# cornellius-gp/linear_operator

Hardware: AMD Instinct MI355X
Metric: cg_member_matvecs_per_sec (higher is better)
Workload: dtype f32

## Files before the change

### linear_operator_amd/csrc/lo_cg_close.h

```cpp
#pragma once
#include "lo_device.h"
#include "lo_internal.h"
#include "lo_cg_onchip.h"
#include "lo_group_reduce.h"

namespace lo {

__device__ __forceinline__ void cg_close_solve(const OnchipArgs& a, const int ngroups, const int t) {
  __shared__ int closer_s;
  __shared__ float red_s[R4_TPB];
  if (t == 0) closer_s = (atomicAdd(a.close_count, 1) == ngroups - 1) ? 1 : 0;
  __syncthreads();
  if (closer_s) {
    float lsum = 0.f, lnan = 0.f, lnotconv = 0.f, lredo = 0.f;
    unsigned spin = 0;
    bool lost = false;
    for (int64_t i = t; i < a.B && !lost; i += R4_TPB) {
      unsigned long long gr;
      for (;;) {
        gr = granule_load(a.close_gran + i);
        if ((granule_tag(gr) & ~7u) == a.close_epoch) break;
        if (++spin > kHandoffMaxSpin || __hip_atomic_load(a.err, __ATOMIC_RELAXED, __HIP_MEMORY_SCOPE_AGENT) != 0) {
          lost = true;
          break;
        }
        __builtin_amdgcn_s_sleep(1);
      }
      if (lost) break;
      const float rn = granule_value(gr);
      const unsigned fl = granule_tag(gr);
      lsum += rn;
      if (rn != rn || (fl & 2u)) lnan = 1.f;
      if (!(fl & 1u)) lnotconv = 1.f;
      if (fl & 4u) lredo = 1.f;
    }
    if (lost) atomicExch(a.err, 1);
    const float mean = block_sum256(lsum, red_s) / (float)a.B;
    const float anynan = block_sum256(lnan, red_s);
    const float notconv = block_sum256(lnotconv, red_s);
    const float redo = block_sum256(lredo, red_s);
    if (t == 0) {
      CgCtrl* c = a.close_ctrl;
      const bool nan = anynan > 0.f;
      const bool skip = !nan && notconv == 0.f;
      const bool tol = !nan && !skip && a.close_floor_ok && mean < a.close_tol;
      c->rs_redo = redo > 0.f ? 1 : 0;
      c->iterations = skip ? 0 : a.iters;
      c->mean_resid = mean;
      c->nan_detected = nan ? 1 : 0;
      c->skipped = skip ? 1 : 0;
      c->tol_reached = tol ? 1 : 0;
      c->stop = (nan || skip || tol) ? 1 : 0;
      c->last_tridiag_iter = 0;
      c->tri_disabled = 0;
      c->oc_err = __hip_atomic_load(a.err, __ATOMIC_RELAXED, __HIP_MEMORY_SCOPE_AGENT);
      if (a.handoff_owned) {
        c->oc_next = c->oc_next_ls = c->pf_next = 0;
        __hip_atomic_store(a.next_member, 0, __ATOMIC_RELAXED, __HIP_MEMORY_SCOPE_AGENT);
        __hip_atomic_store(a.close_count, 0, __ATOMIC_RELAXED, __HIP_MEMORY_SCOPE_AGENT);
      }
      if (a.close_mirror) {
        *a.close_mirror = *c;
        __threadfence_system();
        __hip_atomic_store(reinterpret_cast<unsigned*>(a.close_mirror) + 63, a.close_ticket, __ATOMIC_RELEASE,
                           __HIP_MEMORY_SCOPE_SYSTEM);
      }
    }
  }
}

}
```

### linear_operator_amd/csrc/lo_rspace3.hip

```cpp
#include <algorithm>
#include <atomic>
#include <mutex>
#include <type_traits>
#include <stdlib.h>

#include "lo_device.h"
#include "lo_internal.h"
#include "lo_cg_onchip.h"
#include "lo_group_reduce.h"
#include "lo_cg_close.h"
#include "lo_f64_lanes.h"

namespace lo {

namespace {

typedef float f32x4 __attribute__((ext_vector_type(4)));
typedef __attribute__((address_space(1))) const f32x4 g_cf4;
typedef __attribute__((address_space(1))) const float g_cf;
typedef __attribute__((address_space(1))) float g_f;
typedef __attribute__((address_space(1))) const char g_cc;
template <class T>
__device__ __forceinline__ T* opaque_uniform(T* p) {
  asm volatile("" : "+s"(p));
  return p;
}

constexpr int R3_TPB = 256;
constexpr int R3_ROWS = 1024;

struct PeerOut {
  float* buf[7];
  int n;
  long long member_off;
};
PeerOut g_peer_out = {{nullptr, nullptr, nullptr, nullptr, nullptr, nullptr, nullptr}, 0, 0};
std::mutex g_peer_mu;

__host__ __device__ constexpr int r3_np(int RC) { return 2 * RC + 6; }

__device__ __forceinline__ unsigned xor4_dpp_u(unsigned x) {
  const int a = __builtin_amdgcn_update_dpp(0, (int)x, 0x104, 0xf, 0x5, false);
  return (unsigned)__builtin_amdgcn_update_dpp(a, (int)x, 0x114, 0xf, 0xa, false);
}
__device__ __forceinline__ double halve4_d(double lo, double hi, int lane) {
  const bool up = (lane & 4) != 0;
  const double keep = up ? hi : lo;
  const double send = up ? lo : hi;
  return keep + mk_d(xor4_dpp_u(lo_w(send)), xor4_dpp_u(hi_w(send)));
}

template <int CH>
__device__ __forceinline__ double rows_reduce_d(double (&p)[CH], int lane) {
  if constexpr (CH == 8) {
#pragma unroll
    for (int m = 0; m < 4; ++m) p[m] = halve4_d(p[m], p[m + 4], lane);
    p[0] = halve_pair_d<2>(p[0], p[2], lane);
    p[1] = halve_pair_d<2>(p[1], p[3], lane);
    return halve_pair_d<1>(p[0], p[1], lane);
  } else if constexpr (CH == 4) {
    p[0] = halve_pair_d<2>(p[0], p[2], lane);
    p[1] = halve_pair_d<2>(p[1], p[3], lane);
    return halve_pair_d<1>(p[0], p[1], lane);
  } else {
    return halve_pair_d<1>(p[0], p[1], lane);
  }
}

template <int RC, int GW>
__global__ __launch_bounds__(R3_TPB, 2) void k_cg_rspace3(OnchipArgs a, PeerOut po) {
  constexpr int CH = RC / 4;
  constexpr int RPI = 64 / CH;
  constexpr int NI = 256 / RPI;
  constexpr int NP = r3_np(RC);
  constexpr int MLD = RC + 2;
  constexpr int NH = RC / 2;
  constexpr int NG = 2 * GW * NP;
  __shared__ __attribute__((aligned(16))) float bst[4][256];
  __shared__ __attribute__((aligned(16))) float dst[4][256];
  __shared__ __attribute__((aligned(16))) double mat_s[3 * RC * MLD];
  __shared__ __attribute__((aligned(16))) double red[4][NP];
  __shared__ __attribute__((aligned(16))) double res[NP];
  __shared__ __attribute__((aligned(16))) double gv[4][32];
  __shared__ unsigned polw[GW > 1 ? NG : 2];
  const GroupPlace gp = group_place(GW, (int)gridDim.x / 8);
  if (!gp.active) return;
  const int grp = gp.grp, wig = gp.wig, ngroups = gp.ngroups;
  const int t = threadIdx.x, lane = t & 63, wave = t >> 6;
  const int wave_u = __builtin_amdgcn_readfirstlane(wave);
  unsigned long long* const gbase = a.gbuf + (size_t)grp * 2 * NG;
  unsigned tag = a.tag_base;
  bool same_xcd = false;
  const unsigned xcc = xcc_id();
  bool first = true;
  const int row0 = wig * R3_ROWS + 256 * wave_u;
  const int row0c = max(0, min(row0, a.N - 256));
  const bool di_full = a.dinv_mode == LO_DIAG_FULL;
  float* const bw = bst[wave_u];
  float* const dw = dst[wave_u];
  constexpr int NPF = 8;
  f32x4 pre[NPF];
  constexpr int NXT = NI - NPF;
  f32x4 nxt[NXT > 0 ? NXT : 1];
  auto request = [&](int64_t bm, int tl_, int i_lo, auto cnt, f32x4* dst) {
    const int ln_ = tl_ & 63, k_ = ln_ & (CH - 1), g_ = ln_ / CH;
    const unsigned loff = (unsigned)((g_ * RC + 4 * k_) * sizeof(float));
    g_cc* Cw = (g_cc*)(a.C + ((size_t)bm * a.N + row0c) * RC);
#pragma unroll
    for (int q = 0; q < decltype(cnt)::value / 8; ++q) {
      g_cc* bq = opaque_uniform(Cw + (i_lo + 8 * q + 4) * 1024);
#pragma unroll
      for (int i = 0; i < 8; ++i) dst[8 * q + i] = *(g_cf4*)(bq + loff + (i - 4) * 1024);
    }
  };
  int64_t b = grp;
  {
    int tl0 = t;
    asm volatile("" : "+v"(tl0));
    if (b < a.B) {
      request(b, tl0, 0, std::integral_constant<int, NPF>{}, pre);
      request(b, tl0, NPF, std::integral_constant<int, NXT>{}, nxt);
    } else {
#pragma unroll
      for (int i = 0; i < NPF; ++i) pre[i] = (f32x4){0.f, 0.f, 0.f, 0.f};
    }
  }
  while (b < a.B) {
    const bool stamp = a.dbg && b == a.dbg_member && wig == 0 && t == 0;
    if (stamp) a.dbg[0] = wall_clock64();
    int drawn = 0;
    if (wig == 0 && t == 0) drawn = atomicAdd(a.next_member, 1);
    int tl = t;
    asm volatile("" : "+v"(tl));
    const int ln = tl & 63, k = ln & (CH - 1), g = ln / CH;
    f32x4 Cr[NI];
#pragma unroll
    for (int i = 0; i < NPF; ++i) Cr[i] = pre[i];
#pragma unroll
    for (int i = 0; i < NXT; ++i) Cr[NPF + i] = nxt[i];
    float bq4[4], dq4[4];
    {
      g_cf* bb_ = opaque_uniform((g_cf*)(a.rhs + (size_t)b * a.N + row0c));
      g_cf* dd_ = opaque_uniform((g_cf*)(di_full ? a.dinv + (size_t)b * a.N + row0c : a.dinv + b));
      const int lo_e = row0 - row0c, hi_e = max(0, min(256, a.N - row0c));
      const int dstride = di_full ? 1 : 0;
#pragma unroll
      for (int m = 0; m < 4; ++m) {
        const int e = ln + 64 * m;
        const bool own = e >= lo_e && e < hi_e;
        bq4[m] = own ? bb_[e] : 0.f;
        dq4[m] = own ? dd_[e * dstride] : 0.f;
      }
    }
    constexpr int NM = (3 * RC * RC / 2 + R3_TPB - 1) / R3_TPB;
    f32x4 mv[NM];
    {
      typedef __attribute__((address_space(1))) const f32x4 g_m4;
      const g_m4* src = (const g_m4*)(a.RSD + (size_t)b * 6 * RC * RC);
#pragma unroll
      for (int u = 0; u < NM; ++u) {
        const int e = min(tl + R3_TPB * u, 3 * RC * RC / 2 - 1);
        const int ms = e / (RC * RC / 2);
        const int mg = ms == 0 ? 0 : ms + 1;
        mv[u] = src[(size_t)mg * (RC * RC / 2) + (e - ms * (RC * RC / 2))];
      }
    }
    const double lam_mine = a.RSD[((size_t)b * 6 + 5) * RC * RC + min(ln & 31, RC - 1)];
#pragma unroll
    for (int m = 0; m < 4; ++m) {
      bw[ln + 64 * m] = bq4[m];
      dw[ln + 64 * m] = dq4[m];
    }
#pragma unroll
    for (int u = 0; u < NM; ++u) {
      const int e = tl + R3_TPB * u;
      if (e < 3 * RC * RC / 2) {
        const int mi = e / (RC / 2), jj = e % (RC / 2);
        *reinterpret_cast<f32x4*>(&mat_s[mi * MLD + 2 * jj]) = mv[u];
      }
    }
    __builtin_amdgcn_wave_barrier();
    if (stamp) a.dbg[1] = wall_clock64();

    {
      double aw[4] = {0.0, 0.0, 0.0, 0.0}, au[4] = {0.0, 0.0, 0.0, 0.0};
#pragma unroll
      for (int i0 = 0; i0 < NI; i0 += 4) {
#pragma unroll
        for (int i = i0; i < i0 + 4; ++i) {
          const int r = RPI * i + g;
          const double bb = (double)bw[r];
          const double bd = bb * (double)dw[r];
          const double c0 = (double)Cr[i].x, c1 = (double)Cr[i].y, c2 = (double)Cr[i].z, c3 = (double)Cr[i].w;
          aw[0] = fma(c0, bd, aw[0]); au[0] = fma(c0, bb, au[0]);
          aw[1] = fma(c1, bd, aw[1]); au[1] = fma(c1, bb, au[1]);
          aw[2] = fma(c2, bd, aw[2]); au[2] = fma(c2, bb, au[2]);
          aw[3] = fma(c3, bd, aw[3]); au[3] = fma(c3, bb, au[3]);
        }
        __builtin_amdgcn_sched_barrier(0);
      }
      double s_acc = 0.0, a_acc = 0.0, d2_acc = 0.0;
#pragma unroll
      for (int j = 0; j < 4; ++j) {
        const int rw = 64 * j + RPI * k + g;
        const double bb = (double)bw[rw], di = (double)dw[rw];
        s_acc = fma(bb, bb * di, s_acc);
        a_acc = fma(bb, bb, a_acc);
        d2_acc = fma(di, di, d2_acc);
      }
      double h0 = halve_pair_d<32>(aw[0], au[0], ln), h1 = halve_pair_d<32>(aw[1], au[1], ln);
      double h2 = halve_pair_d<32>(aw[2], au[2], ln), h3 = halve_pair_d<32>(aw[3], au[3], ln);
      h0 = halve_pair_d<16>(h0, h2, ln);
      h1 = halve_pair_d<16>(h1, h3, ln);
      double mine = halve_pair_d<8>(h0, h1, ln);
      if constexpr (CH <= 4) mine = bfly_add_d<4>(mine);
      if constexpr (CH <= 2) mine = bfly_add_d<2>(mine);
      const int comp = (((ln >> 4) & 1) << 1) | ((ln >> 3) & 1);
      const bool writer = (ln & 7 & ~(CH - 1)) == 0;
      if (writer) red[wave_u][((ln >> 5) ? RC : 0) + 4 * k + comp] = mine;
      const double ssum = wave_sum_fast_d(s_acc), asum = wave_sum_fast_d(a_acc), d2sum = wave_sum_fast_d(d2_acc);
      if (ln == 0) {
        red[wave_u][2 * RC] = ssum;
        red[wave_u][2 * RC + 1] = asum;
        red[wave_u][2 * RC + 2] = (wig == 0 && wave_u == 0) ? (double)(ngroups + drawn) : 0.0;
        red[wave_u][2 * RC + 3] = d2sum;
        unsigned xc = xcc;
        asm volatile("" : "+s"(xc));
        red[wave_u][2 * RC + 4] = (first && wave_u == 0) ? (double)xc : 0.0;
        red[wave_u][2 * RC + 5] = (first && wave_u == 0) ? (double)(xc * xc) : 0.0;
      }
    }
#pragma unroll
    for (int i = 0; i < NI; ++i) asm volatile("" : "+v"(Cr[i]));
    __builtin_amdgcn_sched_barrier(0);
    if (a.prefetch & 4) __builtin_amdgcn_s_setprio(3);
    {
      ++tag;
      int tt = (int)threadIdx.x;
      asm volatile("" : "+v"(tt));
      __syncthreads();
      if constexpr (GW == 1) {
        if (tt < NP) res[tt] = (red[0][tt] + red[1][tt]) + (red[2][tt] + red[3][tt]);
      } else {
        unsigned long long* slot = gbase + (size_t)(tag & 1u) * NG;
        if (tt < NP) {
          const double v = (red[0][tt] + red[1][tt]) + (red[2][tt] + red[3][tt]);
          unsigned long long* mine = slot + ((size_t)wig * NP + tt) * 2;
          granule_store(mine, granule_pack_bits(tag, lo_w(v)), same_xcd);
          granule_store(mine + 1, granule_pack_bits(tag, hi_w(v)), same_xcd);
        }
        constexpr int PER = (NG + R3_TPB - 1) / R3_TPB;
        constexpr int CKQ = PER < 8 ? PER : 8;
        unsigned spin = 0;
        bool lost = false;
#pragma unroll 1
        for (int q0 = 0; q0 < PER && !lost; q0 += CKQ) {
          unsigned long long x[CKQ];
          for (;;) {
            bool ok = true;
#pragma unroll
            for (int q = 0; q < CKQ; ++q) {
              const int idx = tt + R3_TPB * (q0 + q);
              x[q] = granule_load(slot + min(idx, NG - 1));
              ok = ok && (granule_tag(x[q]) == tag);
            }
            if (ok) break;
            if (poll_give_up(spin, a.err)) {
              lost = true;
              break;
            }
            __builtin_amdgcn_s_sleep(1);
          }
#pragma unroll
          for (int q = 0; q < CKQ; ++q) {
            const int idx = tt + R3_TPB * (q0 + q);
            if (idx < NG) polw[idx] = granule_bits(x[q]);
          }
        }
        __syncthreads();
        if (tt < NP) {
          double tot = 0.0;
#pragma unroll
          for (int w = 0; w < GW; ++w) tot += mk_d(polw[(w * NP + tt) * 2], polw[(w * NP + tt) * 2 + 1]);
          res[tt] = tot;
        }
      }
      __syncthreads();
    }
    if (GW > 1 && first) {
      unsigned xc = xcc;
      asm volatile("" : "+s"(xc));
      same_xcd = same_xcd_verdict(res[2 * RC + 4], res[2 * RC + 5], GW, xc, a.allow_l2_handoff);
    }
    first = false;
    if (stamp) a.dbg[2] = wall_clock64();
    const int64_t b_next = (int64_t)res[2 * RC + 2];
    {
      int tp = t;
      asm volatile("" : "+v"(tp));
      if (b_next < a.B) {
        request(b_next, tp, 0, std::integral_constant<int, NPF>{}, pre);
      } else {
#pragma unroll
        for (int i = 0; i < NPF; ++i) pre[i] = (f32x4){0.f, 0.f, 0.f, 0.f};
      }
    }
    if (a.prefetch & 1) __builtin_amdgcn_s_setprio(3);

    const int j = lane & 31, hf = lane >> 5;
    const bool live = j < RC;
    const int jr = live ? j : RC - 1;
    double yj = 0.0, xi = 0.0;
    float nrm;
    {
      double a0 = res[2 * RC + 1], s = res[2 * RC];
      const double d2 = res[2 * RC + 3];
      nrm = sqrtf((float)a0);
      const bool rhs_zero = nrm < a.eps;
      if (rhs_zero) nrm = 1.0f;
      const double inv = 1.0 / (double)nrm;
      const double w0 = live ? res[jr] * inv : 0.0, u0 = live ? res[RC + jr] * inv : 0.0;
      s *= inv * inv;
      a0 *= inv * inv;
      float sa = a.stop_after;
      asm volatile("" : "+s"(sa));
      const double sure_rz = 2.0 * (double)sa * (double)sa * sqrt(d2);
      auto own_row_dot = [&](const double* mrow, const double* vec) {
        double a0_ = 0.0, a1_ = 0.0;
#pragma unroll
        for (int q = 0; q < NH; q += 2) {
          const double2 xa = *reinterpret_cast<const double2*>(mrow + q);
          const double2 xx = *reinterpret_cast<const double2*>(vec + q);
          a0_ = fma(xa.x, xx.x, a0_);
          a1_ = fma(xa.y, xx.y, a1_);
        }
        double lo_, up_;
        halves_d(a0_ + a1_, lo_, up_);
        return lo_ + up_;
      };
      double* myv = gv[wave];
      if (hf == 0) myv[j] = w0;
      __builtin_amdgcn_wave_barrier();
      const double* row0m = mat_s + (size_t)jr * MLD + hf * NH;
      double c0 = own_row_dot(row0m, myv + hf * NH);
      double e0 = own_row_dot(row0m + (size_t)1 * RC * MLD, myv + hf * NH);
      const double* nrow = row0m + (size_t)2 * RC * MLD;
      const double* tucol = mat_s + (size_t)(1 * RC + hf * NH) * MLD + jr;
      c0 = live ? c0 : 0.0;
      e0 = live ? e0 : 0.0;
      double tau2 = s - lanes32_sum_d(c0 * e0);
      tau2 = tau2 > 0.0 ? tau2 : 0.0;
      const bool delicate = !rhs_zero && tau2 < 1e-2 * s;
      const double lam = live ? lam_mine : 1.0;
      long long ts_a = 0, ts_b = 0;
      if (stamp) ts_a = wall_clock64();
      double cj = c0, qj = 0.0, etaj = 0.0;
      double cp = 1.0, qp = 0.0, etap = 0.0;
      double rz = 0.0, pApE = 0.0, alpha = 0.0, beta = 0.0;
      float rn = 0.f, last_alpha = 0.f;
      bool conv = false;
      unsigned close_flags = 0u;
      const size_t bc = (size_t)b;
      const bool rec = wig == 0 && lane == 0;
      const int last_owner = (a.iters - 1) & 3;
      for (int kk = -1; kk < a.iters; ++kk) {
        if (kk >= 0) {
          last_alpha = (float)alpha;
          etaj = fma(alpha, qj, etaj);
          etap = fma(alpha, qp, etap);
          cj = fma(-alpha * lam, qj, cj);
          cp = fma(-alpha, qp, cp);
        }
        const double lc = lam * cj;
        const bool lo_h = hf == 0;
        const float inv_rz = __builtin_amdgcn_rcpf((float)rz);
        const double red2 = row16_sum_d(halve_pair_d<16>(lo_h ? cj * cj : lc * qj, lo_h ? lc * cj : 0.0, lane));
        const auto pick = [&](double v, int ln_) {
          return mk_d((unsigned)__builtin_amdgcn_readlane((int)lo_w(v), ln_),
                      (unsigned)__builtin_amdgcn_readlane((int)hi_w(v), ln_));
        };
        const double cc = pick(red2, 0), clc = pick(red2, 16), clq = pick(red2, 32);
        const double rzn = fma(cp * cp, tau2, cc);
        const bool sure = rzn > sure_rz;
        const bool rec_first = kk == 0 && a.close_gran == nullptr && wave == 0;
        const bool rec_last = kk == a.iters - 1 && wave == last_owner;
        const bool own = rec_first || rec_last || !sure;
        float rnn = 0.f;
        if (kk < 0) {
          const float s1f = (float)a0;
          rnn = __builtin_amdgcn_sqrtf(s1f < 0.f ? 0.f : s1f);
        } else if (own) {
          const double dl = fma(-cp, c0, cj);
          __builtin_amdgcn_wave_barrier();
          if (hf == 0) myv[j] = dl;
          __builtin_amdgcn_wave_barrier();
          double gj_;
          {
            double a0_ = 0.0, a1_ = 0.0;
#pragma unroll
            for (int q = 0; q < NH; q += 2) {
              const double2 dd = *reinterpret_cast<const double2*>(myv + hf * NH + q);
              a0_ = fma(tucol[(size_t)q * MLD], dd.x, a0_);
              a1_ = fma(tucol[(size_t)(q + 1) * MLD], dd.y, a1_);
            }
            double lo_, up_;
            halves_d(a0_ + a1_, lo_, up_);
            gj_ = live ? lo_ + up_ : 0.0;
          }
          __builtin_amdgcn_wave_barrier();
          if (hf == 0) myv[j] = gj_;
          __builtin_amdgcn_wave_barrier();
          const double nd = own_row_dot(nrow, myv + hf * NH);
          const double r2 = row16_sum_d(halve_pair_d<16>(gj_ * nd, gj_ * u0, lane));
          const double dnd = pick(r2, 0), dm = pick(r2, 16);
          const double s1 = fma(cp, fma(cp, a0, 2.0 * dm), dnd);
          const float s1f = (float)s1;
          rnn = __builtin_amdgcn_sqrtf(s1f < 0.f ? 0.f : s1f);
        }
        if (kk >= 0) {
          beta = ((float)rz < a.eps) ? 0.0 : (double)((float)rzn * inv_rz);
          if (rhs_zero) rnn = 0.f;
          rn = rnn;
          if (rec && (rec_first || rec_last)) a.resid_rec[(size_t)kk * a.B + bc] = rn;
        } else {
          beta = 0.0;
          rn = rnn;
          if (wig == 0 && t == 0) a.init_conv[bc] = (rn < a.stop_after) ? 1 : 0;
          close_flags = ((rn < a.stop_after) ? 1u : 0u) | (delicate ? 4u : 0u);
          if (delicate && rec && wave == 0) atomicOr(a.err + 4, 1);
        }
        if (kk == 0 && (rnn != rnn || rzn != rzn)) close_flags |= 2u;
        conv = (own || rhs_zero) ? (rn < a.stop_after) : false;
        rz = rzn;
        pApE = fma(beta, fma(beta, pApE, 2.0 * clq), clc);
        qj = fma(beta, qj, cj);
        qp = fma(beta, qp, cp);
        const double pAp = fma(qp * qp, tau2, pApE);
        alpha = ((float)pAp < a.eps) ? 0.0 : (double)((float)rz * __builtin_amdgcn_rcpf((float)pAp));
        if (conv) alpha = 0.0;
      }
      if (stamp) ts_b = wall_clock64();
      if (rec && wave == last_owner) {
        a.rhs_norm[bc] = nrm;
        a.rhs_is_zero[bc] = rhs_zero ? 1 : 0;
        a.rz[bc] = (float)rz;
        a.alpha[bc] = last_alpha;
        a.beta[bc] = (float)beta;
        a.resid_norm[bc] = rn;
        a.has_conv[bc] = conv ? 1 : 0;
        if (a.close_gran) {
          granule_store(a.close_gran + b, granule_pack(a.close_epoch | close_flags, rn), false);
        }
      }
      __builtin_amdgcn_wave_barrier();
      if (hf == 0) myv[j] = fma(-etap, e0, etaj);
      __builtin_amdgcn_wave_barrier();
      xi = etap;
      {
        const double* col = mat_s + (size_t)(hf * NH) * MLD + jr;
        double a0_ = 0.0, a1_ = 0.0;
#pragma unroll
        for (int q = 0; q < NH; q += 2) {
          const double2 ee = *reinterpret_cast<const double2*>(myv + hf * NH + q);
          a0_ = fma(col[(size_t)q * MLD], ee.x, a0_);
          a1_ = fma(col[(size_t)(q + 1) * MLD], ee.y, a1_);
        }
        double lo_, up_;
        halves_d(a0_ + a1_, lo_, up_);
        yj = lo_ + up_;
      }
      yj = live ? yj : 0.0;
      if (stamp) {
        a.dbg[5] = ts_a - a.dbg[2];
        a.dbg[6] = ts_b - ts_a;
        a.dbg[7] = wall_clock64() - ts_b;
      }
      __builtin_amdgcn_wave_barrier();
      if (hf == 0) myv[j] = yj * (double)nrm;
      __builtin_amdgcn_wave_barrier();
    }
    if (!(a.prefetch & 2)) __builtin_amdgcn_s_setprio(0);
    if (stamp) a.dbg[3] = wall_clock64();
    {
      int l2 = lane;
      asm volatile("" : "+v"(l2));
      const int k2 = l2 & (CH - 1), g2 = l2 / CH;
      const double* myv = gv[wave];
      const double2 ya = *reinterpret_cast<const double2*>(&myv[4 * k2]);
      const double2 yb = *reinterpret_cast<const double2*>(&myv[4 * k2 + 2]);
      g_f* const xb = opaque_uniform((g_f*)(a.xout + (size_t)b * a.N + row0c));
      const bool more = b_next < a.B;
      g_cc* const Cn = (g_cc*)(a.C + ((size_t)(more ? b_next : b) * a.N + row0c) * RC);
      const unsigned loffn = (unsigned)((g2 * RC + 4 * k2) * sizeof(float));
#pragma unroll
      for (int js = 0; js < 4; ++js) {
        constexpr int J0 = NPF / CH;
        const int jj = (js + J0) & 3;
        double p[CH];
#pragma unroll
        for (int m = 0; m < CH; ++m) {
          const f32x4 c4 = Cr[CH * jj + m];
          p[m] = fma((double)c4.w, yb.y, fma((double)c4.z, yb.x, fma((double)c4.y, ya.y, (double)c4.x * ya.x)));
        }
        const double xv = rows_reduce_d<CH>(p, l2);
        const int rw = 64 * jj + RPI * k2 + g2;
        const int row = row0c + rw;
        const double acc = fma(xi, (double)bw[rw], xv);
        if (row >= row0 && row < a.N) {
          const float xval = (float)(acc * (double)dw[rw]);
          xb[rw] = xval;
          for (int pp = 0; pp < po.n; ++pp)
            ((g_f*)po.buf[pp])[((size_t)(b + po.member_off)) * a.N + row] = xval;
        }
        if (CH * jj >= NPF) {
          g_cc* bqn = opaque_uniform(Cn + (CH * jj + 4) * 1024);
#pragma unroll
          for (int m = 0; m < CH; ++m)
            nxt[CH * jj - NPF + m] = more ? *(g_cf4*)(bqn + loffn + (m - 4) * 1024) : (f32x4){0.f, 0.f, 0.f, 0.f};
        }
      }
      __builtin_amdgcn_wave_barrier();
    }
    __builtin_amdgcn_s_setprio(0);
    if (stamp) a.dbg[4] = wall_clock64();
    __syncthreads();
    b = b_next;
  }
  if (a.close_gran && wig == 0) cg_close_solve(a, ngroups, t);
}

int rspace3_prio() {
  static const int prio = [] {
    const char* e = getenv("LO_RS_PRIO");
    return e ? atoi(e) : 3;
  }();
  return prio;
}

constexpr size_t HO_MAX_WGS = 2 * 320;
constexpr size_t HO_GRAN_PER_WG = 432;
constexpr size_t HO_MAX_MEMBERS = 65536;
constexpr size_t HO_HEAD_BYTES = 256;
constexpr unsigned HO_TAG_LIMIT = 0xfff00000u;
constexpr unsigned HO_EPOCH_LIMIT = 0x1ffffff0u;
struct HandoffBlock {
  char* buf = nullptr;
  size_t bytes = 0;
  bool failed = false;
  unsigned next_tag = 1, next_epoch = 1;
  unsigned last_launch = 0;
  std::atomic<unsigned> confirmed{0};
  bool force_clear = false;
  unsigned clears = 0, launches = 0;
};
HandoffBlock g_handoff[16];
std::atomic<unsigned> g_handoff_ids{0};

HandoffBlock* handoff_block() {
  int dev = 0;
  if (hipGetDevice(&dev) != hipSuccess || dev < 0 || dev >= 16) return nullptr;
  HandoffBlock& h = g_handoff[dev];
  if (!h.buf && !h.failed) {
    h.bytes = HO_HEAD_BYTES + (HO_MAX_WGS * HO_GRAN_PER_WG + HO_MAX_MEMBERS) * sizeof(unsigned long long);
    if (hipMalloc(&h.buf, h.bytes) != hipSuccess || hipMemset(h.buf, 0, h.bytes) != hipSuccess) {
      (void)hipGetLastError();
      h.buf = nullptr;
      h.failed = true;
    }
  }
  return h.buf ? &h : nullptr;
}

bool handoff_advance(unsigned* next_tag, unsigned* next_epoch, int64_t B, unsigned* tag_base, unsigned* epoch) {
  bool wrap = false;
  const unsigned need = (unsigned)B + 2u;
  if (*next_tag >= HO_TAG_LIMIT - need || *next_epoch >= HO_EPOCH_LIMIT) {
    *next_tag = 1;
    *next_epoch = 1;
    wrap = true;
  }
  *tag_base = *next_tag;
  *epoch = *next_epoch;
  *next_tag += need;
  *next_epoch += 1;
  return wrap;
}

struct OwnedLaunch {
  bool inject;
  unsigned* launch_id;
};

template <int RC, int GW>
int rspace3_go(const OnchipArgs& a, int nwg, const OwnedLaunch* own, hipStream_t st) {
  int per_cu = 0;
  if (LO_OCCUPANCY_CACHED(per_cu, (k_cg_rspace3<RC, GW>), R3_TPB, 0) != hipSuccess || per_cu < 2) return LO_ERR_UNSUPPORTED;
  LO_PROF_BEGIN("cg_onchip", st);
  ResidentLaunch guard(st);
  OnchipArgs a2 = a;
  a2.prefetch = rspace3_prio();
  if (own) {
    hipStreamCaptureStatus cap = hipStreamCaptureStatusNone;
    if (hipStreamIsCapturing(st, &cap) != hipSuccess || cap != hipStreamCaptureStatusNone) {
      (void)hipGetLastError();
      return LO_ERR_UNSUPPORTED;
    }
    HandoffBlock* h = (a.B <= (int64_t)HO_MAX_MEMBERS && (size_t)2 * nwg <= HO_MAX_WGS) ? handoff_block() : nullptr;
    if (!h) return LO_ERR_UNSUPPORTED;
    bool clear = h->force_clear || h->last_launch != h->confirmed.load(std::memory_order_acquire);
    h->force_clear = false;
    clear = handoff_advance(&h->next_tag, &h->next_epoch, a.B, &a2.tag_base, &a2.close_epoch) || clear;
    h->last_launch = g_handoff_ids.fetch_add(1, std::memory_order_relaxed) + 1;
    if (h->last_launch == 0) h->last_launch = g_handoff_ids.fetch_add(1, std::memory_order_relaxed) + 1;
    *own->launch_id = h->last_launch;
    ++h->launches;
    if (clear) {
      ++h->clears;
      const int zrc = zero_span(h->buf, h->bytes, st);
      if (zrc) return zrc;
    }
    a2.close_epoch <<= 3;
    a2.handoff_owned = 1;
    a2.err = reinterpret_cast<int*>(h->buf);
    a2.next_member = a2.err + 1;
    a2.close_count = a2.err + 2;
    a2.gbuf = reinterpret_cast<unsigned long long*>(h->buf + HO_HEAD_BYTES);
    a2.close_gran = a2.gbuf + HO_MAX_WGS * HO_GRAN_PER_WG;
    if (own->inject) LO_HIP_CHECK(hipMemsetAsync(a2.err, 1, 1, st));
  }
  PeerOut po;
  {
    std::lock_guard<std::mutex> lk(g_peer_mu);
    po = g_peer_out;
  }
  hipLaunchKernelGGL((k_cg_rspace3<RC, GW>), dim3(2 * nwg), dim3(R3_TPB), 0, st, a2, po);
  LO_PROF_END(st);
  LO_LAUNCH_CHECK();
  return LO_OK;
}

template <int RC>
int rspace3_gw(const OnchipArgs& a, int nwg, const OwnedLaunch* own, hipStream_t st) {
  switch (a.GW) {
    case 1: return rspace3_go<RC, 1>(a, nwg, own, st);
    case 2: return rspace3_go<RC, 2>(a, nwg, own, st);
    case 4: return rspace3_go<RC, 4>(a, nwg, own, st);
    case 8: return rspace3_go<RC, 8>(a, nwg, own, st);
    case 16: return rspace3_go<RC, 16>(a, nwg, own, st);
    case 32: return rspace3_go<RC, 32>(a, nwg, own, st);
  }
  return LO_ERR_UNSUPPORTED;
}

int rspace3_dispatch(int RC, const OnchipArgs& a, int nwg, const OwnedLaunch* own, hipStream_t st) {
  if (!a.RSD || a.x || a.c != 1 || a.ab_rec || !a.xout || a.GW > 32 || a.N < 256 || (int64_t)a.GW * R3_ROWS < a.N)
    return LO_ERR_UNSUPPORTED;
  if (RC == 32) return rspace3_gw<32>(a, nwg, own, st);
  if (RC == 16) return rspace3_gw<16>(a, nwg, own, st);
  if (RC == 8) return rspace3_gw<8>(a, nwg, own, st);
  return LO_ERR_UNSUPPORTED;
}

}

int rspace3_launch(int RC, const OnchipArgs& a, int nwg, hipStream_t st) { return rspace3_dispatch(RC, a, nwg, nullptr, st); }

int rspace3_launch_owned(int RC, const OnchipArgs& a, int nwg, bool inject, unsigned* launch_id, hipStream_t st) {
  if (!a.close_gran || !a.close_ctrl || !a.close_mirror || a.dbg) return LO_ERR_UNSUPPORTED;
  const OwnedLaunch own = {inject, launch_id};
  return rspace3_dispatch(RC, a, nwg, &own, st);
}

void handoff_launch_confirm(unsigned launch_id) {
  int dev = 0;
  if (hipGetDevice(&dev) != hipSuccess || dev < 0 || dev >= 16) return;
  g_handoff[dev].confirmed.store(launch_id, std::memory_order_release);
}

}

extern "C" int lo_peer_gather_set(float* const* bufs, int n, long long member_offset) {
  if (n < 0 || n > 7 || (n > 0 && !bufs)) return LO_ERR_BADARG;
  std::lock_guard<std::mutex> lk(lo::g_peer_mu);
  for (int i = 0; i < 7; ++i) lo::g_peer_out.buf[i] = i < n ? bufs[i] : nullptr;
  lo::g_peer_out.n = n;
  lo::g_peer_out.member_off = member_offset;
  return LO_OK;
}

extern "C" int lo_resident_handoff_debug(int32_t force_clear, int64_t set_next_tag, int64_t set_next_epoch, uint32_t* out) {
  lo::ResidentLock guard;
  int dev = 0;
  if (hipGetDevice(&dev) != hipSuccess || dev < 0 || dev >= 16) return LO_ERR_BADARG;
  lo::HandoffBlock& h = lo::g_handoff[dev];
  if (set_next_tag > 0xffffffffll || set_next_epoch > 0xffffffffll) return LO_ERR_BADARG;
  if (set_next_tag >= 0) h.next_tag = (unsigned)set_next_tag;
  if (set_next_epoch >= 0) h.next_epoch = (unsigned)set_next_epoch;
  if (force_clear) h.force_clear = true;
  if (out) {
    out[0] = h.next_tag;
    out[1] = h.next_epoch;
    out[2] = h.clears;
    out[3] = h.launches;
  }
  return LO_OK;
}
```

Before: 36.35 million.

## Close CG solve earlier and parallelize closer reduction and control writes

```diff
diff --git a/linear_operator_amd/csrc/lo_cg_close.h b/linear_operator_amd/csrc/lo_cg_close.h
--- a/linear_operator_amd/csrc/lo_cg_close.h
+++ b/linear_operator_amd/csrc/lo_cg_close.h
@@ -1,4 +1,6 @@
 #pragma once
+#include <cstddef>
+
 #include "lo_device.h"
 #include "lo_internal.h"
 #include "lo_cg_onchip.h"
@@ -7,19 +9,36 @@
 namespace lo {
 
 __device__ __forceinline__ void cg_close_solve(const OnchipArgs& a, const int ngroups, const int t) {
+  constexpr int CW = (int)(sizeof(CgCtrl) / sizeof(int));
+  static_assert(sizeof(CgCtrl) == CW * sizeof(int) && CW < 63, "the ticket is word 63 of the pinned block");
   __shared__ int closer_s;
-  __shared__ float red_s[R4_TPB];
+  __shared__ float red_s[R4_WAVES];
+  __shared__ unsigned flag_s[R4_WAVES];
   if (t == 0) closer_s = (atomicAdd(a.close_count, 1) == ngroups - 1) ? 1 : 0;
   __syncthreads();
   if (closer_s) {
-    float lsum = 0.f, lnan = 0.f, lnotconv = 0.f, lredo = 0.f;
+    CgCtrl* c = a.close_ctrl;
+    unsigned keep = 0u;
+    if (t < CW && !a.handoff_owned)
+      keep = __hip_atomic_load(reinterpret_cast<const unsigned*>(c) + t, __ATOMIC_RELAXED, __HIP_MEMORY_SCOPE_AGENT);
+    int err0 = 0;
+    if (t < 64) err0 = __hip_atomic_load(a.err, __ATOMIC_RELAXED, __HIP_MEMORY_SCOPE_AGENT);
+    float lsum = 0.f;
+    unsigned lflags = 0u;
     unsigned spin = 0;
     bool lost = false;
-    for (int64_t i = t; i < a.B && !lost; i += R4_TPB) {
-      unsigned long long gr;
+    constexpr int CK = 4;
+    for (int64_t i0 = t; i0 < a.B && !lost; i0 += CK * R4_TPB) {
+      unsigned long long gr[CK];
       for (;;) {
-        gr = granule_load(a.close_gran + i);
-        if ((granule_tag(gr) & ~7u) == a.close_epoch) break;
+        bool ok = true;
+#pragma unroll
+        for (int q = 0; q < CK; ++q) {
+          const int64_t i = i0 + (int64_t)q * R4_TPB;
+          gr[q] = granule_load(a.close_gran + (i < a.B ? i : a.B - 1));
+          ok = ok && ((granule_tag(gr[q]) & ~7u) == a.close_epoch);
+        }
+        if (ok) break;
         if (++spin > kHandoffMaxSpin || __hip_atomic_load(a.err, __ATOMIC_RELAXED, __HIP_MEMORY_SCOPE_AGENT) != 0) {
           lost = true;
           break;
@@ -27,43 +46,70 @@
         __builtin_amdgcn_s_sleep(1);
       }
       if (lost) break;
-      const float rn = granule_value(gr);
-      const unsigned fl = granule_tag(gr);
-      lsum += rn;
-      if (rn != rn || (fl & 2u)) lnan = 1.f;
-      if (!(fl & 1u)) lnotconv = 1.f;
-      if (fl & 4u) lredo = 1.f;
+#pragma unroll
+      for (int q = 0; q < CK; ++q) {
+        if (i0 + (int64_t)q * R4_TPB < a.B) {
+          const float rn = granule_value(gr[q]);
+          const unsigned fl = granule_tag(gr[q]);
+          lsum += rn;
+          if (rn != rn || (fl & 2u)) lflags |= 1u;
+          if (!(fl & 1u)) lflags |= 2u;
+          if (fl & 4u) lflags |= 4u;
+        }
+      }
     }
-    if (lost) atomicExch(a.err, 1);
-    const float mean = block_sum256(lsum, red_s) / (float)a.B;
-    const float anynan = block_sum256(lnan, red_s);
-    const float notconv = block_sum256(lnotconv, red_s);
-    const float redo = block_sum256(lredo, red_s);
-    if (t == 0) {
-      CgCtrl* c = a.close_ctrl;
-      const bool nan = anynan > 0.f;
-      const bool skip = !nan && notconv == 0.f;
+    if (lost) {
+      atomicExch(a.err, 1);
+      lflags |= 8u;
+    }
+    const float wsum = wave_sum(lsum);
+    const unsigned wflags = (__ballot(lflags & 1u) ? 1u : 0u) | (__ballot(lflags & 2u) ? 2u : 0u) |
+                            (__ballot(lflags & 4u) ? 4u : 0u) | (__ballot(lflags & 8u) ? 8u : 0u);
+    if ((t & 63) == 0) {
+      red_s[t >> 6] = wsum;
+      flag_s[t >> 6] = wflags;
+    }
+    __syncthreads();
+    if (t < 64) {
+      long long nb = a.B;
+      unsigned ticket = a.close_ticket;
+      asm volatile("" : "+s"(nb), "+s"(ticket));
+      const float mean = ((red_s[0] + red_s[1]) + (red_s[2] + red_s[3])) / (float)nb;
+      const unsigned flags = (flag_s[0] | flag_s[1]) | (flag_s[2] | flag_s[3]);
+      const bool nan = (flags & 1u) != 0u;
+      const bool skip = !nan && !(flags & 2u);
       const bool tol = !nan && !skip && a.close_floor_ok && mean < a.close_tol;
-      c->rs_redo = redo > 0.f ? 1 : 0;
-      c->iterations = skip ? 0 : a.iters;
-      c->mean_resid = mean;
-      c->nan_detected = nan ? 1 : 0;
-      c->skipped = skip ? 1 : 0;
-      c->tol_reached = tol ? 1 : 0;
-      c->stop = (nan || skip || tol) ? 1 : 0;
-      c->last_tridiag_iter = 0;
-      c->tri_disabled = 0;
-      c->oc_err = __hip_atomic_load(a.err, __ATOMIC_RELAXED, __HIP_MEMORY_SCOPE_AGENT);
-      if (a.handoff_owned) {
-        c->oc_next = c->oc_next_ls = c->pf_next = 0;
+      const int oc_err = (flags & 8u) ? 1 : err0;
+      unsigned w = keep;
+      bool mine = a.handoff_owned != 0;
+      const auto put = [&](size_t off, unsigned v) {
+        if ((size_t)t * sizeof(int) == off) {
+          w = v;
+          mine = true;
+        }
+      };
+      put(offsetof(CgCtrl, rs_redo), (flags & 4u) ? 1u : 0u);
+      put(offsetof(CgCtrl, iterations), skip ? 0u : (unsigned)a.iters);
+      put(offsetof(CgCtrl, mean_resid), __float_as_uint(mean));
+      put(offsetof(CgCtrl, nan_detected), nan ? 1u : 0u);
+      put(offsetof(CgCtrl, skipped), skip ? 1u : 0u);
+      put(offsetof(CgCtrl, tol_reached), tol ? 1u : 0u);
+      put(offsetof(CgCtrl, stop), (nan || skip || tol) ? 1u : 0u);
+      put(offsetof(CgCtrl, last_tridiag_iter), 0u);
+      put(offsetof(CgCtrl, tri_disabled), 0u);
+      put(offsetof(CgCtrl, oc_err), (unsigned)oc_err);
+      if (t < CW && mine) reinterpret_cast<unsigned*>(c)[t] = w;
+      if (a.handoff_owned && t == 0) {
         __hip_atomic_store(a.next_member, 0, __ATOMIC_RELAXED, __HIP_MEMORY_SCOPE_AGENT);
         __hip_atomic_store(a.close_count, 0, __ATOMIC_RELAXED, __HIP_MEMORY_SCOPE_AGENT);
       }
       if (a.close_mirror) {
-        *a.close_mirror = *c;
+        if (t < CW) reinterpret_cast<unsigned*>(a.close_mirror)[t] = w;
         __threadfence_system();
-        __hip_atomic_store(reinterpret_cast<unsigned*>(a.close_mirror) + 63, a.close_ticket, __ATOMIC_RELEASE,
-                           __HIP_MEMORY_SCOPE_SYSTEM);
+        __builtin_amdgcn_wave_barrier();
+        if (t == 0)
+          __hip_atomic_store(reinterpret_cast<unsigned*>(a.close_mirror) + 63, ticket, __ATOMIC_RELEASE,
+                             __HIP_MEMORY_SCOPE_SYSTEM);
       }
     }
   }
diff --git a/linear_operator_amd/csrc/lo_rspace3.hip b/linear_operator_amd/csrc/lo_rspace3.hip
--- a/linear_operator_amd/csrc/lo_rspace3.hip
+++ b/linear_operator_amd/csrc/lo_rspace3.hip
@@ -113,6 +113,7 @@
       for (int i = 0; i < 8; ++i) dst[8 * q + i] = *(g_cf4*)(bq + loff + (i - 4) * 1024);
     }
   };
+  int closed = 0;
   int64_t b = grp;
   {
     int tl0 = t;
@@ -479,6 +480,14 @@
       if (hf == 0) myv[j] = yj * (double)nrm;
       __builtin_amdgcn_wave_barrier();
     }
+    if (a.close_gran && wig == 0 && po.n == 0 && __builtin_amdgcn_readfirstlane((int)(b_next >= a.B))) {
+      int tc = (int)threadIdx.x;
+      asm volatile("" : "+v"(tc));
+      cg_close_solve(a, ngroups, tc);
+      closed = 1;
+#pragma unroll
+      for (int i = 0; i < NPF; ++i) pre[i] = (f32x4){0.f, 0.f, 0.f, 0.f};
+    }
     if (!(a.prefetch & 2)) __builtin_amdgcn_s_setprio(0);
     if (stamp) a.dbg[3] = wall_clock64();
     {
@@ -526,7 +535,11 @@
     __syncthreads();
     b = b_next;
   }
-  if (a.close_gran && wig == 0) cg_close_solve(a, ngroups, t);
+  if (a.close_gran && wig == 0 && !closed) {
+    int te = (int)threadIdx.x;
+    asm volatile("" : "+v"(te));
+    cg_close_solve(a, ngroups, te);
+  }
 }
 
 int rspace3_prio() {
```

Result: faster. 36.84 million, median of 6 (+1.3%).
